# nebarnix/Project-Desert-Tortoise

Hardware: AMD Instinct MI355X
Metric: IQ Msamples/s end-to-end (WAV→minorframes), 1-GPU + %HBM roofline (higher is better)
Workload: dtype f32

## Files before the change

include/pdt_dev.h:

```cpp
#ifndef PDT_DEV_H
#define PDT_DEV_H
#include <stdint.h>
#ifdef __cplusplus
extern "C" {
#endif
int pdt_dev_set(const char *name, const char *value);
struct pdt_ctx;
unsigned long long pdt_dev_span_rows(const struct pdt_ctx *ctx, unsigned *n_exits_out, unsigned long long max);
unsigned long long pdt_dev_span_rekey(const struct pdt_ctx *ctx, unsigned *out, unsigned long long max);
unsigned pdt_dev_fir_form(const struct pdt_ctx *ctx, unsigned long long *fused_tiles_out);
int pdt_dev_ddc(int device, uint32_t in_rate, int decim, double offset_hz, int sample_format, const void *x_dev, long long lo, long long hi,
                uint64_t n_out, uint64_t g0, void *out_dev);
#ifdef __cplusplus
}
#endif
#endif
```

project-desert-tortoise_amd/__init__.py:

```python
from __future__ import annotations

import collections
import ctypes as C
import os
import struct

import numpy as np

_HERE = os.path.dirname(os.path.abspath(__file__))
LIBPDT_PATH = os.environ.get("PDT_LIBPDT_PATH") or os.path.join(_HERE, "csrc", "libpdt.so")
LIBSYNTH_PATH = os.path.join(_HERE, "synth", "libpdtsynth.so")

MODE_POES, MODE_ARGOS = 0, 1
SAMPLER_GARDNER, SAMPLER_MM = 0, 1
CHAIN_FILE, CHAIN_LIVE = 0, 1
ST_PLL, ST_LOCK, ST_FIR, ST_AGC, ST_SYM, ST_SYMIDX, ST_BITS, ST_BITSYM, ST_AGC_RAW, ST_ANALYTIC, ST_CHANNEL = range(11)
FMT_PCM16, FMT_F32, FMT_REAL_PCM16, FMT_REAL_F32 = range(4)


FMT_WB_PCM16, FMT_WB_F32, FMT_WB_CU8, FMT_WB_CS8 = range(16, 20)


class PdtError(RuntimeError):
    pass
# ... 503 lines not shown
    "pdt_demod_pcm16", "pdt_demod_device", "pdt_demod_f32", "pdt_demod_device_f32", "pdt_demod_batch_device", "pdt_num_frames", "pdt_frames", "pdt_get_stats",
    "pdt_format_frames", "pdt_read_stage", "pdt_stage_len", "pdt_kernel_times", "pdt_make_lpf",
    "pdt_wav_parse_header", "pdt_time_axis", "pdt_stage_bytesync", "pdt_tip_check", "pdt_tip_frames",
    "pdt_stream_begin", "pdt_stream_push_pcm16", "pdt_stream_push_f32", "pdt_stream_end", "pdt_stream_frames",
    "pdt_keep_quality", "pdt_chunk_reports", "pdt_stage_manchester", "pdt_stage_fir", "pdt_stage_agc", "pdt_stage_squelch", "pdt_stage_pll", "pdt_stage_gardner", "pdt_stage_static_gain", "pdt_stage_mm",
    "pdt_keep_presquelch", "pdt_keep_pll", "pdt_stage_bytesync_from", "pdt_demod_fd", "pdt_format_records", "pdt_stream_retained", "pdt_host_math", "pdt_get_device",
    "pdt_write_frames", "pdt_write_records", "pdt_demod_file", "pdt_set_loop_params", "pdt_set_progress",
    "pdt_set_real_input", "pdt_demod_real", "pdt_demod_device_real", "pdt_stream_push_real", "pdt_host_analytic",
    "pdt_set_channel", "pdt_demod_channel", "pdt_demod_device_channel", "pdt_demod_channels_device", "pdt_demod_channels", "pdt_stream_push_channel", "pdt_host_ddc",
    "pdt_survey", "pdt_survey_device", "pdt_survey_spectrum", "pdt_host_survey",
    "pdt_bursts", "pdt_bursts_device", "pdt_burst_carriers", "pdt_waterfall_rows", "pdt_bursts_shape", "pdt_burst_peaks", "pdt_host_bursts",
    "pdt_device_math", "pdt_device_math_layout",
    "pdt_burst_windows", "pdt_demod_windows_device", "pdt_demod_windows", "pdt_demod_windows_held",
    "pdt_tones", "pdt_tones_batch", "pdt_host_tones",
    "pdt_argos_messages", "pdt_argos_messages_batch", "pdt_stage_argos_messages", "pdt_host_argos_messages", "pdt_argos_msg_tile",
    "pdt_format_argos_messages", "pdt_write_argos_messages",
    "pdt_ff_bits", "pdt_ff_bits_batch", "pdt_ff_read", "pdt_ff_messages", "pdt_ff_messages_batch", "pdt_stage_ff_bits", "pdt_host_ff_bits",
    "pdt_host_ff_mix",
    "pdt_ffp_bits", "pdt_ffp_read", "pdt_ffp_blocks", "pdt_ffp_frames", "pdt_stage_ffp_bits", "pdt_stage_ffp_frames", "pdt_host_ffp_bits",
    "pdt_host_ffp_mix",
    "pdt_tip_sync", "pdt_tip_sync_batch", "pdt_stage_tip_sync", "pdt_host_tip_sync", "pdt_tip_sync_tile", "pdt_tip_check_records",
    "pdt_tip_repair", "pdt_stage_tip_repair", "pdt_host_tip_repair",
]
DEV_SYMBOLS = ["pdt_dev_set", "pdt_dev_span_rows", "pdt_dev_span_rekey", "pdt_dev_fir_form", "pdt_dev_ddc"]

_lib = None


def _share_torch_hip_runtime():
    import importlib.util
    import sys
    if "torch" in sys.modules:
        return
    try:
        spec = importlib.util.find_spec("torch")
    except (ImportError, ValueError):
        return
    if spec is None or not spec.submodule_search_locations:
        return
    path = os.path.join(list(spec.submodule_search_locations)[0], "lib", "libamdhip64.so")
    if os.path.exists(path):
        try:
            C.CDLL(path, mode=C.RTLD_GLOBAL)
        except OSError:
            pass


# ... 63 lines not shown
    L.pdt_stage_mm.argtypes = [C.c_void_p, C.c_void_p, C.c_uint64, C.c_void_p, C.c_void_p, C.c_void_p, C.c_void_p]
    L.pdt_stage_mm.restype = C.c_int
    L.pdt_stage_agc.argtypes = [C.c_void_p, C.c_void_p, C.c_uint64, C.c_double, C.c_double, C.c_double, C.c_void_p]
    L.pdt_stage_agc.restype = C.c_int
    L.pdt_stage_squelch.argtypes = [C.c_void_p, C.c_void_p, C.c_void_p, C.c_uint64, C.c_double]
    L.pdt_stage_squelch.restype = C.c_int
    L.pdt_stage_fir.argtypes = [C.c_void_p, C.c_void_p, C.c_uint64, C.c_void_p, C.c_void_p]
    L.pdt_stage_fir.restype = C.c_int
    L.pdt_keep_quality.argtypes = [C.c_void_p, C.c_int]
    L.pdt_keep_quality.restype = C.c_int
    L.pdt_keep_pll.argtypes = [C.c_void_p, C.c_int]
    L.pdt_keep_pll.restype = C.c_int
    L.pdt_chunk_reports.argtypes = [C.c_void_p, C.c_void_p, C.c_uint64]
    L.pdt_chunk_reports.restype = C.c_uint64
    L.pdt_set_progress.argtypes = [C.c_void_p, C.c_void_p, C.c_void_p]
    L.pdt_tip_check.argtypes = [C.c_void_p, C.POINTER(TipSummary)]
    L.pdt_tip_frames.argtypes = [C.c_void_p, C.c_void_p, C.c_uint64]
    L.pdt_tip_frames.restype = C.c_uint64
    L.pdt_write_frames.argtypes = [C.c_void_p, C.c_int, C.POINTER(C.c_uint64)]
    L.pdt_write_records.argtypes = [C.c_void_p, C.c_uint64, C.c_int, C.POINTER(C.c_uint64)]
    L.pdt_dev_set.argtypes = [C.c_char_p, C.c_char_p]
    L.pdt_dev_fir_form.argtypes = [C.c_void_p, C.POINTER(C.c_ulonglong)]
    L.pdt_dev_fir_form.restype = C.c_uint
    L.pdt_set_loop_params.argtypes = [C.c_void_p, C.POINTER(LoopParams)]
    L.pdt_demod_file.argtypes = [C.c_void_p, C.c_int, C.c_uint64, C.c_uint64, C.c_int, C.c_int, C.POINTER(C.c_uint64)]
    L.pdt_set_real_input.argtypes = [C.c_void_p, C.c_double]
    L.pdt_demod_real.argtypes = [C.c_void_p, C.c_void_p, C.c_uint64, C.c_int]
    L.pdt_demod_device_real.argtypes = [C.c_void_p, C.c_void_p, C.c_uint64, C.c_int]
    L.pdt_stream_push_real.argtypes = [C.c_void_p, C.c_void_p, C.c_uint64, C.c_int, C.POINTER(C.c_uint64)]
    L.pdt_host_analytic.argtypes = [C.c_uint32, C.c_double, C.c_void_p, C.c_uint64, C.c_int, C.c_void_p]
    L.pdt_set_channel.argtypes = [C.c_void_p, C.c_int, C.c_double]
    L.pdt_demod_channel.argtypes = [C.c_void_p, C.c_void_p, C.c_uint64, C.c_int]
    L.pdt_demod_device_channel.argtypes = [C.c_void_p, C.c_void_p, C.c_uint64, C.c_int]
    L.pdt_demod_channels_device.argtypes = [C.POINTER(C.c_void_p), C.c_int, C.c_void_p, C.c_uint64, C.c_int]
    L.pdt_demod_channels.argtypes = [C.POINTER(C.c_void_p), C.c_int, C.c_void_p, C.c_uint64, C.c_int]
    L.pdt_stream_push_channel.argtypes = [C.c_void_p, C.c_void_p, C.c_uint64, C.c_int, C.POINTER(C.c_uint64)]
    L.pdt_host_ddc.argtypes = [C.c_uint32, C.c_int, C.c_double, C.c_void_p, C.c_uint64, C.c_int, C.c_void_p]
    L.pdt_dev_ddc.argtypes = [C.c_int, C.c_uint32, C.c_int, C.c_double, C.c_int, C.c_void_p, C.c_longlong, C.c_longlong, C.c_uint64, C.c_uint64, C.c_void_p]
    L.pdt_survey.argtypes = [C.c_void_p, C.c_void_p, C.c_uint64, C.c_int, C.POINTER(SurveyCfg), C.POINTER(CarrierRec), C.c_int, C.POINTER(C.c_int)]
    L.pdt_survey_device.argtypes = L.pdt_survey.argtypes
    L.pdt_survey_spectrum.argtypes = [C.c_void_p, C.c_void_p, C.c_int]
    L.pdt_bursts.argtypes = [C.c_void_p, C.c_void_p, C.c_uint64, C.c_int, C.POINTER(BurstsCfg), C.POINTER(BurstRec), C.c_int, C.POINTER(C.c_int)]
    L.pdt_bursts_device.argtypes = L.pdt_bursts.argtypes
    L.pdt_burst_carriers.argtypes = [C.POINTER(BurstRec), C.c_int, C.c_double, C.POINTER(CarrierRec), C.c_int, C.POINTER(C.c_int)]
    L.pdt_waterfall_rows.argtypes = [C.c_void_p, C.c_uint64, C.c_uint64, C.c_void_p]
    L.pdt_bursts_shape.argtypes = [C.c_void_p, C.POINTER(C.c_int), C.POINTER(C.c_int), C.POINTER(C.c_uint64)]
# ... 523 lines not shown
        ns = C.c_uint64(0)
        _check(self._L.pdt_stage_mm(self._h, a.ctypes.data, a.size, C.addressof(state) if state is not None else None,
                                    sym.ctypes.data, pick.ctypes.data, C.addressof(ns)), "pdt_stage_mm")
        return sym[:ns.value], pick[:ns.value]

    def stage_agc(self, x: np.ndarray, initial: float, state: "AgcState | None" = None, attack: float = 0.0, decay: float = 0.0):
        a = np.array(x, dtype=self._dt(), copy=True)
        _check(self._L.pdt_stage_agc(self._h, a.ctypes.data, a.size, float(initial), float(attack), float(decay),
                                     C.addressof(state) if state is not None else None), "pdt_stage_agc")
        return a

    def stage_squelch(self, x: np.ndarray, lock: np.ndarray, threshold: float) -> np.ndarray:
        a = np.array(x, dtype=self._dt(), copy=True)
        l = np.ascontiguousarray(lock, dtype=self._dt())
        assert a.size == l.size
        _check(self._L.pdt_stage_squelch(self._h, a.ctypes.data, l.ctypes.data, a.size, float(threshold)), "pdt_stage_squelch")
        return a

    def fir_form(self) -> "tuple[int, int]":
        tiles = C.c_ulonglong(0)
        form = self._L.pdt_dev_fir_form(self._h, C.byref(tiles))
        return int(form), int(tiles.value)

    def stats_interp(self) -> int:
        taps, interp = make_lpf(self.mode, self.sample_rate)
        return int(interp)

    def frames(self) -> list[Frame]:
        n = self._L.pdt_num_frames(self._h)
        arr = (Frame * max(n, 1))()
        got = self._L.pdt_frames(self._h, arr, n)
        return [arr[i] for i in range(got)]

    def frames_array(self) -> np.ndarray:
        n = self._L.pdt_num_frames(self._h)
        buf = np.zeros(n, dtype=FRAME_DTYPE)
        if n:
            self._L.pdt_frames(self._h, C.cast(buf.ctypes.data, C.POINTER(Frame)), n)
        return buf

    def stats(self) -> Stats:
        s = Stats()
        _check(self._L.pdt_get_stats(self._h, C.byref(s)), "pdt_get_stats")
        return s

    def text(self) -> bytes:
# ... 265 lines not shown
```

project-desert-tortoise_amd/csrc/pdt_api.hip:

```cpp
#include "pdt_rt.h"
#include "pdt_analytic.h"
#include "pdt_ddc.h"
#include "pdt_survey.h"
#include "pdt_bursts.h"
#include "pdt_tone.h"
#include "pdt_argos_msg.h"
#include "pdt_tip_sync.h"
#include "pdt_ff.h"
#include "pdt_ffp.h"

#include <sys/stat.h>

namespace pdtrt {
PDT_CHAIN_INSTANCES(extern, float)
PDT_CHAIN_INSTANCES(extern, double)
std::atomic<long long> g_alloc_ns{0};
hipError_t analytic_launch(hipStream_t st, int fmt, const void *x, long long lo, long long hi, unsigned long long n_out, unsigned long long g0,
                           uint32_t step, const float *tab_dev, void *out);
size_t survey_part_floats(uint64_t nseg, int nfft);
hipError_t survey_launch(hipStream_t st, int fmt, const void *x, uint64_t nseg, int nfft, const float *win, const float *tw, float *part, float *out);
int survey_plan(const pdt_survey_cfg *cfg, double mode_range_hz, double channel_rate, uint64_t nframes, int cap, pdt::SurveyPlan *p);
int survey_carriers(const float *P, const pdt::SurveyPlan &p, double in_rate, pdt_carrier *found);
hipError_t waterfall_launch(hipStream_t st, int fmt, const void *x, uint64_t nrows, int rows_per, int nfft, const float *win, const float *tw, float *rows);
hipError_t row_peaks_launch(hipStream_t st, const float *rows, uint64_t nrows, int nfft, float level, int gb, void *peaks, int *counts);
// ... 21 lines not shown
               std::vector<uint32_t> &starts, pdt::FfpSync *head);
hipError_t tip_repair_launch(hipStream_t st, void *recs_dev, unsigned nrec, const float *soft_dev, const unsigned long long *nbits_dev, long long bit_cap,
                             void *info_dev, void *sum_dev);
long long ddc_windows_table(int decim, pdt::DdcWindow *win, int count, std::vector<unsigned char> &table);
hipError_t ddc_windows_launch(hipStream_t st, int fmt, int decim, const float *taps_dev, const float *tab_dev, const void *table_dev, int count,
                              long long tiles);
hipError_t ddc_launch(hipStream_t st, int fmt, int decim, const float *taps_dev, const float *tab_dev, pdt::DdcWindow w);
}

static std::mutex g_dev_mu;
static std::map<std::string, std::string> g_dev;
void Tuning::load()
{
    std::lock_guard<std::mutex> lock(g_dev_mu);
    if (g_dev.empty()) return;
    auto get = [&](const char *n) -> const char * { auto it = g_dev.find(n); return it == g_dev.end() ? nullptr : it->second.c_str(); };
    if (const char *e = get("PDT_PLL_WARM_SCALE")) pll_warm_scale = atof(e);
    if (const char *e = get("PDT_HEAD_TAUS")) head_taus = atof(e);
    if (const char *e = get("PDT_BAND_PAD")) band_pad = atof(e);
    if (const char *e = get("PDT_PLL_WARM_S")) pll_warm_s = atof(e);
    if (const char *e = get("PDT_AGC_WARM_S")) agc_warm_s = atof(e);
    if (const char *e = get("PDT_AGC_K")) agc_k = atof(e);
    if (const char *e = get("PDT_AGC_TPB")) agc_tpb = std::max(1, atoi(e));
    if (const char *e = get("PDT_PLL_BLOCK")) pll_block = atoi(e);
    if (const char *e = get("PDT_HBM_LIMIT_MB")) hbm_limit_mb = std::max(1ll, atoll(e));
    if (const char *e = get("PDT_BURST_SLAB_ROWS")) burst_slab_rows = std::max(1ll, atoll(e));
    if (const char *e = get("PDT_WINDOW_PIECE")) window_piece = std::max(1ll, atoll(e));
    if (const char *e = get("PDT_SCOUT_SYMS")) scout_syms = std::max(16, atoi(e));
    if (const char *e = get("PDT_FIR_WG_PER_CU")) fir_wg_per_cu = std::min(4096, std::max(1, atoi(e)));
    if (const char *e = get("PDT_INGEST_THREADS")) ingest_threads = std::min(128, std::max(1, atoi(e)));
    if (const char *e = get("PDT_INGEST_SPAN_MB")) ingest_span_mb = std::min(256, std::max(1, atoi(e)));
    if (const char *e = get("PDT_INGEST_STREAMS")) ingest_streams = std::min(4, std::max(1, atoi(e)));
    if (const char *e = get("PDT_INGEST_DIRECT")) ingest_direct = atoi(e) ? 1 : 0;
    if (const char *e = get("PDT_INGEST_NUMA")) ingest_numa = atoi(e) ? 1 : 0;
    if (const char *e = get("PDT_FIX_PASSES")) fix_passes = atoi(e);
    if (const char *e = get("PDT_GSEG")) gseg = std::min(64, std::max(2, atoi(e)));
    if (const char *e = get("PDT_GSPAN")) gspan = std::min(256, std::max(1, atoi(e)));
    if (const char *e = get("PDT_GSPAN_REKEY")) gspan_rekey = std::min(255, std::max(0, atoi(e)));
    if (const char *e = get("PDT_GSPAN_SUB")) gspan_sub = atoi(e);
    if (const char *e = get("PDT_GSPAN_WIN2")) gspan_win2 = atoi(e);
    if (const char *e = get("PDT_GSPAN_FIT")) gspan_fit = std::min(64, std::max(2, atoi(e)));
    if (const char *e = get("PDT_GSPAN_CAP")) gspan_cap = std::max(64, atoi(e));
    fir_generic = get("PDT_FIR_GENERIC") != nullptr;
    mix_unfused = get("PDT_MIX_UNFUSED") != nullptr;
    quality_inline = get("PDT_QUALITY_INLINE") != nullptr;
    gardner_nostride = get("PDT_GARDNER_NOSTRIDE") != nullptr;
// ... 228 lines not shown
    if (out && m) {
        const bool staged = ctx->gspan_rekey > 0 && ctx->gspan_info.p;
        std::vector<GardnerSpanRow> rows((size_t)m);
        std::vector<GardnerSpanRowInfo> info((size_t)m);
        if (hipSetDevice(ctx->cfg.device) != hipSuccess ||
            hipMemcpy(rows.data(), ctx->gspan_rows.p, (size_t)m * sizeof(GardnerSpanRow), hipMemcpyDeviceToHost) != hipSuccess ||
            (staged && hipMemcpy(info.data(), ctx->gspan_info.p, (size_t)m * sizeof(GardnerSpanRowInfo), hipMemcpyDeviceToHost) != hipSuccess)) {
            (void)hipGetLastError();
            return 0;
        }
        for (size_t k = 0; k < (size_t)m; k++) {
            out[3 * k] = rows[k].n;
            out[3 * k + 1] = staged ? info[k].states : 0u;
            out[3 * k + 2] = staged ? info[k].items : 0u;
        }
    }
    return n;
}

unsigned pdt_dev_fir_form(const pdt_ctx *ctx, unsigned long long *fused_tiles_out)
{
    if (fused_tiles_out) *fused_tiles_out = ctx ? (unsigned long long)ctx->fir_fused_tiles : 0ull;
    return ctx ? (unsigned)ctx->fir_form : 0u;
}

int pdt_dev_ddc(int device, uint32_t in_rate, int decim, double offset_hz, int sample_format, const void *x_dev, long long lo, long long hi,
                uint64_t n_out, uint64_t g0, void *out_dev)
{
    if (in_rate == 0 || decim < DDC_MIN_DECIM || decim > DDC_MAX_DECIM || !ddc_fmt(sample_format) || !x_dev || !out_dev) return PDT_ERR_ARG;
    if (!(std::isfinite(offset_hz) && std::fabs(offset_hz) < 0.5 * (double)in_rate)) return PDT_ERR_ARG;
    HIP_TRY(hipSetDevice(device));
    const std::vector<float> taps = ddc_taps(decim);
    std::vector<float> tab(2 * AN_TAB);
    analytic_table(tab.data());
    DevBuf dtaps, dtab;
    auto run = [&]() -> int {
        int rc;
        if ((rc = dtaps.ensure(taps.size() * sizeof(float) + 16)) || (rc = dtab.ensure(tab.size() * sizeof(float) + 16))) return rc;
        HIP_TRY(hipMemcpy(dtaps.p, taps.data(), taps.size() * sizeof(float), hipMemcpyHostToDevice));
        HIP_TRY(hipMemcpy(dtab.p, tab.data(), tab.size() * sizeof(float), hipMemcpyHostToDevice));
        const DdcWindow r = { x_dev, out_dev, lo, hi, (long long)n_out, ddc_step((double)in_rate, offset_hz), (uint32_t)g0, 0 };
        HIP_TRY(ddc_launch(nullptr, sample_format, decim, (const float *)dtaps.p, (const float *)dtab.p, r));
        HIP_TRY(hipStreamSynchronize(nullptr));
        return PDT_OK;
    };
    const int rc = run();
// ... 2676 lines not shown
```

project-desert-tortoise_amd/csrc/pdt_chain.inc:

```
#include "pdt_rt.h"

namespace pdtrt {
PDT_WIDE_INSTANCES(extern, float)
PDT_WIDE_INSTANCES(extern, double)

template <typename T> int finish_capture(pdt_ctx *ctx, uint64_t n, const FinishArgs &FA)
{
    const bool argos = FA.argos, need_lock = FA.need_lock, fuse_mix = FA.fuse_mix;
    const long long N = FA.N, n_out = FA.n_out, chunk = FA.chunk, chunk_out = FA.chunk_out, first = FA.first, first_out = FA.first_out,
                    sym_cap = FA.sym_cap;
    const int interp = FA.interp, ntaps = FA.ntaps;
    const uint32_t hit_cap = FA.hit_cap, frame_cap = FA.frame_cap;
    const SyncParams &SP = FA.SP;
    const T Fs = (T)ctx->cfg.sample_rate;
    StreamCarry *seg = ctx->sc.active ? &ctx->sc : nullptr;
    FrameRec *d_frames = (FrameRec *)ctx->frames.p;
    (void)first_out;
    if (!ctx->pending || ctx->pend_n != n) return PDT_ERR_STATE;
    ctx->pending = false;
    pdt_ctx *lead = ctx->leader ? ctx->leader : ctx;
    if (seg && seg->in_place && !ctx->tune.sync_block) {
        for (;;) {
            const hipError_t e = hipEventQuery(lead->ev1);
            if (e == hipSuccess) break;
// ... 243 lines not shown

    collect_timers();
    if (ctx->progress_fn && !ctx->chunk_host.empty()) {
        try {
            std::vector<pdt_chunk_report> rep(ctx->chunk_host.size());
            chunk_reports_range(ctx, 0, rep.size(), ctx->report_samples, rep.data(), nullptr);
            ctx->progress_fn(ctx->progress_user, 0, rep.data(), rep.size(), &ctx->stats);
        } catch (const std::bad_alloc &) {
            return PDT_ERR_NOMEM;
        }
    }
    return PDT_OK;
}


inline void agc_block_warm(const pdt_ctx *ctx, long long *Ba, long long *Wa)
{
    const bool argos = ctx->cfg.mode == PDT_MODE_ARGOS;
    const double fs_d = (double)ctx->cfg.sample_rate;
    const int interp = (int)ctx->interp;
    auto round4 = [](long long v) { return (v + 3) / 4 * 4; };
    *Ba = std::max<long long>(64, round4(ctx->cfg.agc_block ? ctx->cfg.agc_block : (long long)((argos ? 0.125 : 0.0625) * fs_d * interp)));
    *Wa = round4(ctx->cfg.agc_warm ? ctx->cfg.agc_warm : (long long)((argos ? 2.0 : 8.0) * fs_d * interp));
}

template <typename T> void rec_static_gain(Plan &PL, hipStream_t st, IqSrc src, long long n, T *mag, T level, double norm_override, T *d_norm)
{
    PDT_LAUNCH(256, k_static_gain<T>, dim3(1), dim3(256), 0, st, src, n, mag, level, norm_override, d_norm);
}

template <typename T> void rec_squelch(Plan &PL, hipStream_t st, T *data, const T *lock, long long n, T thr)
{
    PDT_LAUNCH(256, k_squelch<T>, dim3((unsigned)((n + 1023) / 1024)), dim3(256), 0, st, data, lock, n, thr);
}

template <typename T> bool rec_fir_unfused(pdt_ctx *ctx, Plan &PL, hipStream_t st, const T *d_in, long long N, T *d_out, AgcMap *tile_maps, T agc_decay)
{
    const bool argos = ctx->cfg.mode == PDT_MODE_ARGOS;
    const int interp = (int)ctx->interp, ntaps = (int)ctx->ntaps;
    const T *d_taps = (const T *)ctx->taps.p;
    const int opt = 8;
    const long long tile = (long long)PDT_FIR_THREADS * opt;
    const long long grid = (N * interp + tile - 1) / tile;
    if (argos) {
        const size_t sh = (size_t)(ntaps + tile + ntaps + 8) * sizeof(T);
        PDT_LAUNCH(PDT_FIR_THREADS, k_fir_plain<T>, dim3((unsigned)grid), dim3(PDT_FIR_THREADS), sh, st, d_in, N, ntaps, d_taps, d_out, opt);
// ... 265 lines not shown
        Wacq = (long long)(0.02 * fs_d);
        agc_block_warm(ctx, &Ba, &Wa);
        if (argos && !ctx->cfg.agc_block && ctx->batch_hint >= 8) Ba = (long long)(1.0 * fs_d * interp);
        if (!ctx->cfg.pll_block) {
            const long long groups_max = ctx->batch_hint > 1 ? 240 : 150;
            const long long share = std::max<long long>(1, groups_max / std::max(1, ctx->batch_hint));
            const long long b_min = (N + share * 256 - 1) / (share * 256);
            Bp = std::max(Bp, b_min);
        }
        Bp = std::min<long long>(Bp, std::max<long long>(N, 1));
        Bp = std::max<long long>(64, (Bp + 63) / 64 * 64);
        seg_fast = seg && first_out % PDT_MF_RUN == 0 && first_out % 32 == 0 && !ctx->tune.seg_plain;
        fuse_mix = false;
        if constexpr (std::is_same<T, float>::value) {
            fuse_mix = !argos && !live && !inject && (!seg || seg_fast) && interp == 1 && ntaps == 26 && ctx->taps_rot.p && !ctx->tune.fir_generic &&
                       !ctx->tune.mix_unfused && N >= 832;
            if (fuse_mix && !ctx->cfg.pll_block) Bp = (Bp + 831) / 832 * 832;
            if (fuse_mix && Bp % 832 != 0) fuse_mix = false;
        }
        Ba = std::max<long long>(64, round4(Ba));
        agc_tiles_per_block = 0;
        fused_tiles = 0;
        agc_maps_per_block = 0;
        if (!argos && !ctx->cfg.agc_block && ntaps == 26 * interp && ctx->taps_rot.p && !ctx->tune.fir_generic &&
            !ctx->tune.agc_unfused && (!seg || (seg_fast && first_out % (64ll * 26 * interp) == 0) || (seg_fast && fuse_mix))) {
            const long long tile_out = 64ll * 26 * interp;
            agc_tiles_per_block = std::max<long long>(1, (Ba + tile_out / 2) / tile_out);
            {
                const long long tiles = (n_out - first_out + tile_out - 1) / tile_out;
                const long long one_round = (tiles + 500ll * 64 - 1) / (500ll * 64);
                if (ctx->batch_hint <= 1 && tiles / agc_tiles_per_block > 512ll * 64 && one_round <= 4 * agc_tiles_per_block)
                    agc_tiles_per_block = one_round;
            }
            if (ctx->tune.agc_tpb) agc_tiles_per_block = ctx->tune.agc_tpb;
            Ba = agc_tiles_per_block * tile_out;
        }
        Wp = round4(Wp);
        Wa = round4(Wa);
        Wacq = round4(Wacq);
        sym_rate = (double)baud;
        f_lim = (double)PP.max_freq * fs_d / (2.0 * M_PI);
        lag = (int)ceil(fs_d / sym_rate);
        lag = std::max(1, std::min(lag, (int)(fs_d / (2.2 * f_lim))));
        lag = std::min(lag, 64);
        nb_pll = N / Bp + 2;
        nb_agc = (n_out - first_out + Ba - 1) / Ba + 1;

        return PDT_OK;
    }

    int allocate()
    {
        int rc = PDT_OK;
        (void)rc;
        min_step = (double)GP.step - 0.25;
        if (ctx->cfg.sampler == PDT_SAMPLER_MM) {
            if ((rc = make_mm_params<T>(ctx, n_out, chunk_out, nullptr))) return rc;
// ... 385 lines not shown
                    else PDT_LAUNCH(512, (k_mix_fir<26, 1, 8, true>), dim3(mf_grid), dim3(512), 0, st, PDT_MF_ARGS, d_tap, mf_pll_from);
                } else {
                    if (d_pcm.fmt == 0) PDT_LAUNCH(512, (k_mix_fir<26, 0, 8>), dim3(mf_grid), dim3(512), 0, st, PDT_MF_ARGS, (float *)nullptr, mf_pll_from);
                    else PDT_LAUNCH(512, (k_mix_fir<26, 1, 8>), dim3(mf_grid), dim3(512), 0, st, PDT_MF_ARGS, (float *)nullptr, mf_pll_from);
                }
#undef PDT_MF_ARGS
                done = true;
            }
            if (!done) done = rec_fir_unfused<T>(ctx, PL, st, (const T *)d_pll, N, d_fir, fir_tile_maps, AP.decay);
            if (!done) fused_tiles = 0;
            ctx->fir_form = fuse_mix ? 2 : done ? 3 : argos ? 1 : 4;
            L.end();
        }
        ctx->fir_fused_tiles = fused_tiles;

        return PDT_OK;
    }

    int rec_agc()
    {
        int rc = PDT_OK;
        (void)rc;
        agc_last_block = -1;
        if (n_out - first_out > 0) {
            const long long na = n_out - first_out;
            const T *a_in = d_fir + first_out;
            T *a_out = d_agc + first_out;
            const T *a_lock = d_lock ? d_lock + first_out : nullptr;
            AgcParams<T> APs = AP;
            if (APs.raw_out) APs.raw_out += first_out;
            const long long nb = (na + Ba - 1) / Ba;
            agc_last_block = nb - 1;
            const bool fused = fused_tiles > 0;
            if (!fused && (rc = ctx->agc_maps.ensure((size_t)(nb + 1) * (sizeof(AgcMap) + sizeof(double))))) return rc;
            AgcMap *d_maps = (AgcMap *)ctx->agc_maps.p;
            double *d_guess = (double *)(d_maps + (fused ? fused_tiles : nb) + 1);
            const long long map_len_fused = fuse_mix ? (long long)PDT_MF_RUN : 64ll * 26 * interp;
            const long long map_first = fused ? first_out / map_len_fused : 0;
            const AgcMap *d_maps_in = d_maps + map_first;
            const long long n_maps_in = fused ? fused_tiles - map_first : nb;
            if (quality_side && !quality_term_fused) PL.simple(OP_JOIN_WAIT);
            L.begin("agc_block");
            if (agc_maps_per_block == 0) agc_maps_per_block = agc_tiles_per_block;
            if (fused && agc_maps_per_block > 1) {
                AgcMap *d_bmaps = (AgcMap *)(d_guess + nb + 1);
                PDT_LAUNCH(256, k_agc_blockmaps, dim3((unsigned)((nb + 255) / 256)), dim3(256), 0, st, d_maps_in, nb,
                                   (int)agc_maps_per_block, n_maps_in, d_bmaps);
                PDT_LAUNCH(1024, k_agc_guess<T>, dim3(1), dim3(1024), 0, st, (const AgcMap *)d_bmaps, nb, (const T *)d_norm, d_guess, 1, nb);
            } else if (fused)
                PDT_LAUNCH(1024, k_agc_guess<T>, dim3(1), dim3(1024), 0, st, d_maps_in, nb, (const T *)d_norm, d_guess, (int)agc_maps_per_block, n_maps_in);
            bool agc_tr = false;
            float *agc_ckpt = nullptr;
            if constexpr (std::is_same<T, float>::value) {
                agc_tr = fused && !ctx->tune.agc_lanes && !APs.squelch && !APs.raw_out && first_out % 32 == 0 && Ba % 32 == 0 &&
                         agc_maps_per_block > 0 && Ba % agc_maps_per_block == 0;
                if (agc_tr) {
                    const long long tile_len = 64ll * 26 * interp;
                    const long long map_len = Ba / agc_maps_per_block;
                    agc_tr = tile_len % 32 == 0 && tile_len % map_len == 0 && Ba % tile_len == 0;
                    if (agc_tr) {
                        const double agc_K = ctx->tune.agc_k > 0 ? ctx->tune.agc_k : 12.0;
                        const size_t ck_bytes = (size_t)(nb + 64) * (size_t)(Ba / PDT_AGC_CKPT + 1) * sizeof(float);
                        if ((rc = ctx->agc_ckpt.ensure(ck_bytes))) return rc;
                        agc_ckpt = (float *)ctx->agc_ckpt.p;
                        PDT_LAUNCH(64, (k_agc_block_tr<PDT_AGC_TR_R>), dim3((unsigned)((nb + 63) / 64)), dim3(64), 0, st, (const float *)a_in, na, APs,
                                   (const float *)d_norm, Ba, Wa, (const double *)d_guess, d_maps_in, (int)agc_maps_per_block,
                                   (int)(tile_len / map_len), n_maps_in, tile_len, (float *)a_out, (AgcSeam<float> *)ctx->seams_agc.p, agc_K, agc_ckpt);
                    }
                }
            }
            T *agc_ckpt_any = (T *)agc_ckpt;
            if (!agc_tr && (rc = rec_agc_lanes<T>(ctx, PL, st, a_in, na, APs, d_norm, Ba, Wa, !fused, d_maps, d_guess, a_lock, a_out, &agc_ckpt_any))) return rc;
            L.end();
            L.begin("agc_fix");
            rec_agc_fix<T>(ctx, PL, st, a_in, na, APs, Ba, a_lock, a_out, d_sc, agc_ckpt_any);
            L.end();
        }

        return PDT_OK;
    }

    int sampler_domain()
    {
        int rc = PDT_OK;
        (void)rc;
        use_mm = ctx->cfg.sampler == PDT_SAMPLER_MM;
        use_table = false;
        GD.q_min = 0; GD.u = 0; GD.n_q = 0; GD.n_cand = 0; GD.pad_q = 0; GD.idx_bits = 20; GD.span = 1;
        span_rekey = 0;
        if constexpr (std::is_same<T, float>::value) {
// ... 775 lines not shown
```

project-desert-tortoise_amd/csrc/pdt_kernels_front.h:

```cpp
#pragma once
#include <type_traits>
#include <utility>
#include "pdt_device_math.h"

namespace pdt {

template <typename T> struct PllParams {
    T Fs;
    T lock_thr;
    T lock_alpha;
    T alpha_acq, beta_acq, alpha_trk, beta_trk;
    T alpha_wide, beta_wide;
    T max_freq, min_freq;
    T sweep0, avg0, phase0;
    T freq0, locksig0;
    long long i0;
    T cond_lo, cond_hi;
    int want_lock;
};

template <typename T> struct PllState {
    T phase, freq, avg_phase, locksig, sweep;
};

// ... 2376 lines not shown
            __syncthreads();
            if ((int)threadIdx.x >= d) {
                Bc = A * Bp + Bc;
                A = A * Ap;
                sA[threadIdx.x] = A;
                sB[threadIdx.x] = Bc;
            }
            __syncthreads();
        }
        if (threadIdx.x == 0) {
            const double tA = sA[255], tB = sB[255];
            runB = tA * runB + tB;
            runA = tA * runA;
        }
    }
    if (threadIdx.x == 0) {
        AgcMap m;
        m.A = runA;
        m.B = runB;
        maps[j] = m;
    }
}

__device__ __forceinline__ void k_agc_blockmaps(const AgcMap *__restrict__ maps, long long nb, int maps_per_block, long long n_maps,
                                                AgcMap *__restrict__ bmaps)
{
    const long long j = (long long)blockIdx.x * blockDim.x + threadIdx.x;
    if (j >= nb) return;
    AgcMap bm;
    bm.A = 1.0; bm.B = 0.0;
    for (int q = 0; q < maps_per_block; q++) {
        const long long t = j * maps_per_block + q;
        if (t < n_maps) {
            const AgcMap m = maps[t];
            bm.B = m.A * bm.B + m.B;
            bm.A = m.A * bm.A;
        }
    }
    bmaps[j] = bm;
}

template <typename T>
__device__ __forceinline__ void k_agc_guess(const AgcMap *__restrict__ maps, long long nb, const T *__restrict__ norm,
                                                     double *__restrict__ guesses, int maps_per_block, long long n_maps)
{
    __shared__ double sA[1024], sB[1024];
    const long long per = (nb + 1023) / 1024;
    long long j0 = (long long)threadIdx.x * per, j1 = j0 + per;
    if (j0 > nb) j0 = nb;
    if (j1 > nb) j1 = nb;
    auto block_map = [&](long long j) {
        AgcMap bm;
        bm.A = 1.0; bm.B = 0.0;
        for (int q = 0; q < maps_per_block; q++) {
            const long long t = j * maps_per_block + q;
            if (t < n_maps) {
                const AgcMap m = maps[t];
                bm.B = m.A * bm.B + m.B;
                bm.A = m.A * bm.A;
            }
        }
        return bm;
    };
    double A = 1.0, Bc = 0.0;
    for (long long j = j0; j < j1; j++) {
        const AgcMap m = block_map(j);
        Bc = m.A * Bc + m.B;
        A = m.A * A;
    }
    sA[threadIdx.x] = A;
    sB[threadIdx.x] = Bc;
    __syncthreads();
    for (int d = 1; d < 1024; d <<= 1) {
        double Ap = 1.0, Bp = 0.0;
        if ((int)threadIdx.x >= d) { Ap = sA[threadIdx.x - d]; Bp = sB[threadIdx.x - d]; }
        __syncthreads();
        if ((int)threadIdx.x >= d) {
            Bc = A * Bp + Bc;
            A = A * Ap;
            sA[threadIdx.x] = A;
            sB[threadIdx.x] = Bc;
        }
        __syncthreads();
    }
    double Ae = 1.0, Be = 0.0;
    if (threadIdx.x > 0) { Ae = sA[threadIdx.x - 1]; Be = sB[threadIdx.x - 1]; }
    double g = Ae * (double)*norm + Be;
    for (long long j = j0; j < j1; j++) {
        double gg = g;
        if (!(gg > 1e-4)) gg = 1e-4;
        if (gg > 5000.0) gg = 5000.0;
        guesses[j] = gg;
        const AgcMap m = block_map(j);
        g = m.A * g + m.B;
    }
}

#define PDT_AGC_CKPT 1024
template <typename T>
__device__ __forceinline__ void k_agc_block(const T *__restrict__ in, long long n, AgcParams<T> P,
                                                   const T *__restrict__ norm, long long B, long long W,
                                                   const double *__restrict__ guesses, const T *__restrict__ lock,
                                                   T *__restrict__ out, AgcSeam<T> *__restrict__ seams, double K,
                                                   T *__restrict__ ckpt )
{
    __shared__ __attribute__((aligned(16))) unsigned char ring[PDT_AGC_PF * PDT_RING_SLOT];
    const long long j = (long long)blockIdx.x * blockDim.x + threadIdx.x;
    const long long start = j * B;
    if (start >= n) return;
    const long long end = (start + B < n) ? start + B : n;
    long long ws = 0;
    T gain = *norm;
    if (j >= 1) {
        const double g_here = guesses[j];
        double need = K * g_here / (double)P.decay;
        if (need < 4096.0) need = 4096.0;
        if (need > (double)W) need = (double)W;
        long long m = (long long)((need + (double)B - 1.0) / (double)B);
// ... 4 lines not shown
            gain = (T)g0;
        }
    }
    agc_range<T, false>(in, lock, out, ws, start, gain, P, ring);
    AgcSeam<T> sm;
    sm.g0 = gain;
    if (ckpt) {
        const long long ncp = B / PDT_AGC_CKPT;
        long long at = start;
        for (long long c = 0; c < ncp && at + PDT_AGC_CKPT <= end; c++, at += PDT_AGC_CKPT) {
            agc_range<T, true>(in, lock, out, at, at + PDT_AGC_CKPT, gain, P, ring);
            ckpt[j * ncp + c] = gain;
        }
        agc_range<T, true>(in, lock, out, at, end, gain, P, ring);
    } else
        agc_range<T, true>(in, lock, out, start, end, gain, P, ring);
    sm.g1 = gain;
    seams[j] = sm;
}

#define PDT_TR_SLOT 1040
#define PDT_TR_SB (8 * PDT_TR_SLOT)
#ifndef PDT_AGC_TR_R
#define PDT_AGC_TR_R 4
#endif
typedef float pdt_f4 __attribute__((ext_vector_type(4)));

template <bool STORE, bool PARTIAL, bool CLAMP, int R>
__device__ __forceinline__ void agc_range_tr(const float *__restrict__ in, float *__restrict__ out, long long e0, int rel0, long long nsb,
                                             float &gain, int from, const AgcParams<float> &P, unsigned char *ring,
                                             const unsigned (&voff)[8], long long n, long long B, long long jb0,
                                             float *__restrict__ ckpt = nullptr)
{
    const int t = threadIdx.x & 63;
    const unsigned ring0 = (unsigned)(size_t)ring;
    const unsigned char *mine = ring + (t & 7) * PDT_TR_SLOT + (t >> 3) * 128;
    unsigned char *stage_mine = ring + R * PDT_TR_SB + (t & 7) * PDT_TR_SLOT + (t >> 3) * 128;
    const unsigned char *stage_row = ring + R * PDT_TR_SB + t * 16;
    const char *gin = (const char *)(in + e0);
    char *gout = (char *)(out + e0);
    auto issue = [&](long long sb, int slot) {
        const char *b = gin + sb * 128;
#pragma unroll
        for (int s = 0; s < 8; s++) {
            unsigned vo = voff[s];
            if (CLAMP) {
                const long long e = e0 + sb * 32;
// ... 87 lines not shown
    const long long j = jb0 + t;
    const long long start = j * B;
    const bool valid = start < n;
    unsigned voff[8];
#pragma unroll
    for (int s = 0; s < 8; s++) {
        long long b = 8 * (t >> 3) + s;
        if ((jb0 + b) * B >= n) b = 0;
        voff[s] = (unsigned)((b * B + 4 * (t & 7)) * 4);
    }
    long long ws = 0;
    float gain = *norm;
    if (valid && j >= 1) {
        const double g_here = guesses[j];
        double need = K * g_here / (double)P.decay;
        if (need < 4096.0) need = 4096.0;
        if (need > (double)W) need = (double)W;
        const long long m = (long long)((need + (double)tile_len - 1.0) / (double)tile_len);
        const long long q = (start - m * tile_len) / tile_len;
        if (start - m * tile_len > 0 && q >= 1) {
            ws = q * tile_len;
            const long long jb = ws / B;
            double g = guesses[jb];
            for (long long u = jb * maps_per_block; u < q * maps_per_tile; u++)
                if (u < n_maps) {
                    const AgcMap mp = tmaps[u];
                    g = mp.A * g + mp.B;
                }
            if (!(g > 1e-4)) g = 1e-4;
            if (g > 5000.0) g = 5000.0;
            gain = (float)g;
        }
    }
    const bool partial = (jb0 + 64) * B > n;
    int back = valid ? (int)(start - ws) : 0;
#pragma unroll
    for (int d = 32; d >= 1; d >>= 1) {
        const int o = __shfl_xor(back, d);
        back = back > o ? back : o;
    }
    back = __builtin_amdgcn_readfirstlane(back);
    const int from = valid ? -(int)(start - ws) : 0x7fffffff;
    if (back > 0) {
        if (jb0 * B >= back) agc_range_tr<false, false, false, R>(in, out, jb0 * B - back, -back, back / 32, gain, from, P, ring, voff, n, B, jb0);
        else agc_range_tr<false, false, true, R>(in, out, jb0 * B - back, -back, back / 32, gain, from, P, ring, voff, n, B, jb0);
    }
    AgcSeam<float> sm;
    sm.g0 = gain;
    float *my_ckpt = (ckpt && valid) ? ckpt + j * (B / PDT_AGC_CKPT) : nullptr;
    if (!partial) agc_range_tr<true, false, false, R>(in, out, jb0 * B, 0, B / 32, gain, 0, P, ring, voff, n, B, jb0, my_ckpt);
    else agc_range_tr<true, true, false, R>(in, out, jb0 * B, 0, B / 32, gain, 0, P, ring, voff, n, B, jb0, my_ckpt);
// ... 73 lines not shown
```

project-desert-tortoise_amd/csrc/pdt_rt.h:

```cpp
#ifndef PDT_RT_H
#define PDT_RT_H
#include <hip/hip_runtime.h>
#include <math.h>
#include <stdio.h>
#include <stdlib.h>
#include <string.h>

#include <errno.h>
#include <fcntl.h>
#include <unistd.h>

#include <algorithm>
#include <functional>
#include <map>
#include <mutex>
#include <atomic>
#include <chrono>
#include <memory>
#include <new>
#include <string>
#include <thread>
#include <type_traits>
#include <vector>

#include "../../include/pdt.h"
#include "../../include/pdt_dev.h"
#include "pdt_kernels_back.h"
#include "pdt_kernels_front.h"
#include "pdt_timeaxis.h"
#include "pdt_ingest.h"
#include "pdt_work_layout.h"

using namespace pdt;

#define HIP_TRY(expr)                                                                                  \
    do {                                                                                               \
        hipError_t e_ = (expr);                                                                        \
        if (e_ != hipSuccess) {                                                                        \
            fprintf(stderr, "libpdt: %s failed: %s (%s:%d)\n", #expr, hipGetErrorString(e_), __FILE__, \
                    __LINE__);                                                                         \
            return PDT_ERR_NOGPU;                                                                      \
        }                                                                                              \
    } while (0)

namespace pdtrt {

extern std::atomic<long long> g_alloc_ns;
struct AllocTimer {
    std::chrono::steady_clock::time_point t0 = std::chrono::steady_clock::now();
    ~AllocTimer() { g_alloc_ns += std::chrono::duration_cast<std::chrono::nanoseconds>(std::chrono::steady_clock::now() - t0).count(); }
};
inline hipError_t timed_host_malloc(void **p, size_t bytes)
{
    AllocTimer t;
// ... 175 lines not shown
    bool same_shape(const Plan &o) const
    {
        if (ops.size() != o.ops.size() || packs.size() != o.packs.size()) return false;
        for (size_t i = 0; i < ops.size(); i++) {
            const PlanOp &a = ops[i], &b = o.ops[i];
            if (a.op != b.op || a.side != b.side || a.go != b.go || a.block.x != b.block.x || a.block.y != b.block.y ||
                a.shmem != b.shmem || a.pack_off != b.pack_off || a.pack_size != b.pack_size)
                return false;
        }
        return true;
    }
};
#define PDT_LAUNCH(TB, KERNEL, grid, block, shmem, stream, ...) \
    PL.launch<&KERNEL, TB>(#KERNEL, grid, block, shmem, PL.side_of(stream), __VA_ARGS__)

}
using namespace pdtrt;

struct Tuning {
    double band_pad = 0.0, pll_warm_scale = 1.0, head_taus = 0.0, agc_k = 0.0, pll_warm_s = 0.0, agc_warm_s = 0.0;
    double overlap_split[8] = { 0, 0, 0, 0, 0, 0, 0, 0 };
    long long hbm_limit_mb = 0, window_piece = 0, burst_slab_rows = 0;
    int ingest_direct = -1, ingest_numa = -1;
    int scout_syms = 0, gspan = 0, gspan_cap = 0, gspan_rekey = -1 , gspan_sub = 0, gspan_win2 = 0, gspan_fit = 0, ingest_threads = 0, ingest_span_mb = 0, ingest_streams = 0, overlap_segments = 0, overlap_min_mb = 0, fir_wg_per_cu = 0, agc_tpb = 0, gseg = 0, pll_block = 0, fix_passes = 2;
    bool fir_generic = false, mix_unfused = false, quality_inline = false, gemit_groups = false, agc_unfused = false, no_excl = false, gardner_onebuf = false, gardner_noring = false, gardner_sequential = false, seg_sequential = false, agc_lanes = false, overlap = true, debug_overlap = false, chain_one_range = false, ema_noguess = false, debug_sync = false, pll_noshort = false, pll_nockpt = false, pll_noconsensus = false, pll_notail = false, seg_plain = false, sync_block = false, gardner_nostride = false, manch_3pass = false, sync_serial = false;
    void load();
};

struct StreamCarry {
    bool active = false;
    bool final_seg = false;
    bool in_place = false;
    uint64_t place_align = 0;
    bool quality = false;
    long long first = 0;
    uint64_t origin = 0;
    bool have_norm = false;
    double norm_factor = 0, gain = 0;
    bool locked = false;
    double phase = 0, freq = 0, avg = 0, locksig = 0, sweep = 0;
    int64_t lock_sample = -1;
    double lock_freq_hz = 0, avg_at_lock = 0;
    bool have_sampler = false;
    double sa = 0, sb = 0, sc = 0;
    double sym_m2 = 0, sym_m1 = 0;
    unsigned clockmod = 0;
    uint64_t nsym_total = 0;
// ... 64 lines not shown
    bool keep_agc_raw = false;
    bool keep_quality = false;
    bool keep_pll_asked = false;
    bool keep_pll = true;
    DevBuf avgph, term_ap, seams_q, chunkinfo;
    struct PllInject {
        bool active = false, started = false, locked = false;
        double phase = 0, freq = 0, avg = 0, locksig = 0, sweep = 0;
    } inj;
    long long last_pll_block = 0;
    void *qual_pin = nullptr;
    size_t qual_pin_cap = 0;
    uint64_t pend_chunks = 0;
    std::vector<pdt::ChunkInfo> chunk_host;
    uint64_t report_samples = 0;
    pdt_progress_fn progress_fn = nullptr;
    void *progress_user = nullptr;
    long long gcand_key = -1;
    int gardner_mode = 0;
    long long gspan_nrows = 0;
    int gspan_rekey = 0;
    int fir_form = 0;
    long long fir_fused_tiles = 0;
    const void *pcm_dev = nullptr;
    int pcm_fmt = 0;

    std::vector<unsigned char> taps_host;
    uint64_t n_samples = 0, n_out = 0;
    std::vector<pdt_frame> frames_host;
    std::vector<pdt_tip_frame> tip_host;
    uint32_t frames_on_device = 0;
    bool have_frames = false;
    Plan plan;
    DevBuf packs_dev;
    void *packs_pin = nullptr;
    size_t packs_pin_cap = 0;
    pdt_ctx *leader = nullptr;
    int batch_hint = 1;
    IngestRes ingest;
    double stream_gpu_ms = 0;
    double ingest_ms = 0;
    DevBuf stream_in, seg_dev, lt_theta, lt_phi;
    uint64_t stream_have = 0, stream_done = 0;
    uint64_t stream_total = 0;
    int stream_fmt = -1;
    bool stream_open = false;
    std::vector<pdt_frame> stream_new;
    uint32_t real_step = 1u << 30;
    double real_center = 0;
    DevBuf an_tab, analytic;
    int an_tab_ready = 0;
    uint64_t analytic_len = 0;
    int ch_decim = 0;
    double ch_offset = 0;
    uint32_t ch_step = 0;
    DevBuf ddc_taps, channel;
    int ddc_taps_decim = 0;
    uint64_t channel_len = 0;
    HaloCarry halo;
    DevBuf survey_win, survey_tw, survey_part, survey_out;
    int survey_tab_nfft = 0;
// ... 388 lines not shown
```

Measured before the change: 55270.

## Size AGC tiles-per-block from device LDS occupancy and shrink transpose ring depth

Sets the AGC tiles-per-block split from queried CU count and LDS capacity, taking walkers per round from the kernel's static LDS size. It replaces the hard-coded 500/512×64 lane heuristic. The default transpose ring depth drops from 4 to 3, adding a runtime switch that instantiates depths 3–5. Map-composition loops are batched eight loads at a time. The aim is a better-balanced single-round AGC sweep with more resident workgroups, at the cost of less prefetch depth per walker.

Result: no change. 55350, median of 4 (+0.2%).

```diff
diff --git a/include/pdt_dev.h b/include/pdt_dev.h
--- a/include/pdt_dev.h
+++ b/include/pdt_dev.h
@@ -9,6 +9,7 @@
 unsigned long long pdt_dev_span_rows(const struct pdt_ctx *ctx, unsigned *n_exits_out, unsigned long long max);
 unsigned long long pdt_dev_span_rekey(const struct pdt_ctx *ctx, unsigned *out, unsigned long long max);
 unsigned pdt_dev_fir_form(const struct pdt_ctx *ctx, unsigned long long *fused_tiles_out);
+unsigned pdt_dev_agc_form(const struct pdt_ctx *ctx, unsigned long long *tiles_per_block_out, unsigned long long *walkers_out);
 int pdt_dev_ddc(int device, uint32_t in_rate, int decim, double offset_hz, int sample_format, const void *x_dev, long long lo, long long hi,
                 uint64_t n_out, uint64_t g0, void *out_dev);
 #ifdef __cplusplus
diff --git a/project-desert-tortoise_amd/__init__.py b/project-desert-tortoise_amd/__init__.py
--- a/project-desert-tortoise_amd/__init__.py
+++ b/project-desert-tortoise_amd/__init__.py
@@ -549,7 +549,7 @@
     "pdt_tip_sync", "pdt_tip_sync_batch", "pdt_stage_tip_sync", "pdt_host_tip_sync", "pdt_tip_sync_tile", "pdt_tip_check_records",
     "pdt_tip_repair", "pdt_stage_tip_repair", "pdt_host_tip_repair",
 ]
-DEV_SYMBOLS = ["pdt_dev_set", "pdt_dev_span_rows", "pdt_dev_span_rekey", "pdt_dev_fir_form", "pdt_dev_ddc"]
+DEV_SYMBOLS = ["pdt_dev_set", "pdt_dev_span_rows", "pdt_dev_span_rekey", "pdt_dev_fir_form", "pdt_dev_agc_form", "pdt_dev_ddc"]
 
 _lib = None
 
@@ -659,6 +659,8 @@
     L.pdt_dev_set.argtypes = [C.c_char_p, C.c_char_p]
     L.pdt_dev_fir_form.argtypes = [C.c_void_p, C.POINTER(C.c_ulonglong)]
     L.pdt_dev_fir_form.restype = C.c_uint
+    L.pdt_dev_agc_form.argtypes = [C.c_void_p, C.POINTER(C.c_ulonglong), C.POINTER(C.c_ulonglong)]
+    L.pdt_dev_agc_form.restype = C.c_uint
     L.pdt_set_loop_params.argtypes = [C.c_void_p, C.POINTER(LoopParams)]
     L.pdt_demod_file.argtypes = [C.c_void_p, C.c_int, C.c_uint64, C.c_uint64, C.c_int, C.c_int, C.POINTER(C.c_uint64)]
     L.pdt_set_real_input.argtypes = [C.c_void_p, C.c_double]
@@ -1228,6 +1230,11 @@
         form = self._L.pdt_dev_fir_form(self._h, C.byref(tiles))
         return int(form), int(tiles.value)
 
+    def agc_form(self) -> "tuple[int, int, int]":
+        tpb, walkers = C.c_ulonglong(0), C.c_ulonglong(0)
+        ring = self._L.pdt_dev_agc_form(self._h, C.byref(tpb), C.byref(walkers))
+        return int(ring), int(tpb.value), int(walkers.value)
+
     def stats_interp(self) -> int:
         taps, interp = make_lpf(self.mode, self.sample_rate)
         return int(interp)
diff --git a/project-desert-tortoise_amd/csrc/pdt_agc_geometry.h b/project-desert-tortoise_amd/csrc/pdt_agc_geometry.h
--- /dev/null
+++ b/project-desert-tortoise_amd/csrc/pdt_agc_geometry.h
@@ -0,0 +1,36 @@
+#ifndef PDT_AGC_GEOMETRY_H
+#define PDT_AGC_GEOMETRY_H
+
+namespace pdtrt {
+
+enum { AGC_SIMDS_PER_CU = 4, AGC_LANES = 64 };
+
+inline long long agc_walkers_per_cu(long long lds_per_cu, long long lds_per_wg)
+{
+    if (lds_per_wg <= 0) return AGC_SIMDS_PER_CU;
+    const long long fit = lds_per_cu / lds_per_wg;
+    return fit < 0 ? 0 : fit > AGC_SIMDS_PER_CU ? AGC_SIMDS_PER_CU : fit;
+}
+
+enum { AGC_WALKERS_PER_CU_PACED = 2 };
+
+inline long long agc_walkers_per_round(long long cus, long long lds_per_cu, long long lds_per_wg)
+{
+    const long long fit = agc_walkers_per_cu(lds_per_cu, lds_per_wg);
+    return cus <= 0 ? 0 : cus * (fit > AGC_WALKERS_PER_CU_PACED ? AGC_WALKERS_PER_CU_PACED : fit);
+}
+
+inline long long agc_tiles_per_block(long long walkers, long long tiles, long long tpb_default, long long forced)
+{
+    if (forced > 0) return forced;
+    if (tpb_default < 1) tpb_default = 1;
+    if (walkers <= 0 || tiles <= 0) return tpb_default;
+    const long long lanes_full = walkers * AGC_LANES;
+    const long long lanes = walkers * 125 / 128 * AGC_LANES > 0 ? walkers * 125 / 128 * AGC_LANES : lanes_full;
+    const long long one_round = (tiles + lanes - 1) / lanes;
+    if (tiles / tpb_default > lanes_full && one_round <= 4 * tpb_default) return one_round;
+    return tpb_default;
+}
+
+}
+#endif
diff --git a/project-desert-tortoise_amd/csrc/pdt_api.hip b/project-desert-tortoise_amd/csrc/pdt_api.hip
--- a/project-desert-tortoise_amd/csrc/pdt_api.hip
+++ b/project-desert-tortoise_amd/csrc/pdt_api.hip
@@ -67,6 +67,7 @@
     if (const char *e = get("PDT_AGC_WARM_S")) agc_warm_s = atof(e);
     if (const char *e = get("PDT_AGC_K")) agc_k = atof(e);
     if (const char *e = get("PDT_AGC_TPB")) agc_tpb = std::max(1, atoi(e));
+    if (const char *e = get("PDT_AGC_RING")) agc_ring = std::min(5, std::max(3, atoi(e)));
     if (const char *e = get("PDT_PLL_BLOCK")) pll_block = atoi(e);
     if (const char *e = get("PDT_HBM_LIMIT_MB")) hbm_limit_mb = std::max(1ll, atoll(e));
     if (const char *e = get("PDT_BURST_SLAB_ROWS")) burst_slab_rows = std::max(1ll, atoll(e));
@@ -341,6 +342,13 @@
 {
     if (fused_tiles_out) *fused_tiles_out = ctx ? (unsigned long long)ctx->fir_fused_tiles : 0ull;
     return ctx ? (unsigned)ctx->fir_form : 0u;
+}
+
+unsigned pdt_dev_agc_form(const pdt_ctx *ctx, unsigned long long *tiles_per_block_out, unsigned long long *walkers_out)
+{
+    if (tiles_per_block_out) *tiles_per_block_out = ctx ? (unsigned long long)ctx->agc_form_tpb : 0ull;
+    if (walkers_out) *walkers_out = ctx ? (unsigned long long)ctx->agc_form_walkers : 0ull;
+    return ctx ? (unsigned)ctx->agc_form_ring : 0u;
 }
 
 int pdt_dev_ddc(int device, uint32_t in_rate, int decim, double offset_hz, int sample_format, const void *x_dev, long long lo, long long hi,
diff --git a/project-desert-tortoise_amd/csrc/pdt_chain.inc b/project-desert-tortoise_amd/csrc/pdt_chain.inc
--- a/project-desert-tortoise_amd/csrc/pdt_chain.inc
+++ b/project-desert-tortoise_amd/csrc/pdt_chain.inc
@@ -289,6 +289,34 @@
     auto round4 = [](long long v) { return (v + 3) / 4 * 4; };
     *Ba = std::max<long long>(64, round4(ctx->cfg.agc_block ? ctx->cfg.agc_block : (long long)((argos ? 0.125 : 0.0625) * fs_d * interp)));
     *Wa = round4(ctx->cfg.agc_warm ? ctx->cfg.agc_warm : (long long)((argos ? 2.0 : 8.0) * fs_d * interp));
+}
+
+static_assert(PDT_AGC_TR_R >= 3 && PDT_AGC_TR_R <= 5, "k_agc_block_tr is instantiated for ring depths 3, 4 and 5");
+inline int agc_ring_depth(const pdt_ctx *ctx) { return ctx->tune.agc_ring ? ctx->tune.agc_ring : PDT_AGC_TR_R; }
+
+template <int R> long long agc_tr_static_lds()
+{
+    hipFuncAttributes fa;
+    if (hipFuncGetAttributes(&fa, reinterpret_cast<const void *>(&k_run<&k_agc_block_tr<R>, 64>)) != hipSuccess) {
+        (void)hipGetLastError();
+        return (long long)(R + 1) * PDT_TR_SB;
+    }
+    return (long long)fa.sharedSizeBytes;
+}
+template <typename T> long long agc_round_walkers(pdt_ctx *ctx, int R)
+{
+    if (!std::is_same<T, float>::value) R = 0;
+    long long &have = ctx->agc_round_walkers[R ? R - 2 : 0];
+    if (have > 0) return have;
+    int cus = 0, lds_cu = 0, lds_wg = 0;
+    if (hipDeviceGetAttribute(&cus, hipDeviceAttributeMultiprocessorCount, ctx->cfg.device) != hipSuccess) { (void)hipGetLastError(); cus = 0; }
+    if (hipDeviceGetAttribute(&lds_cu, hipDeviceAttributeMaxSharedMemoryPerMultiprocessor, ctx->cfg.device) != hipSuccess) { (void)hipGetLastError(); lds_cu = 0; }
+    if (hipDeviceGetAttribute(&lds_wg, hipDeviceAttributeMaxSharedMemoryPerBlock, ctx->cfg.device) != hipSuccess) { (void)hipGetLastError(); lds_wg = 0; }
+    long long lds = (long long)PDT_AGC_PF * PDT_RING_SLOT;
+    if constexpr (std::is_same<T, float>::value)
+        lds = R == 3 ? agc_tr_static_lds<3>() : R == 4 ? agc_tr_static_lds<4>() : R == 5 ? agc_tr_static_lds<5>() : lds;
+    have = agc_walkers_per_round(cus, std::max(lds_cu, lds_wg), lds);
+    return have;
 }
 
 template <typename T> void rec_static_gain(Plan &PL, hipStream_t st, IqSrc src, long long n, T *mag, T level, double norm_override, T *d_norm)
@@ -600,17 +628,19 @@
         agc_tiles_per_block = 0;
         fused_tiles = 0;
         agc_maps_per_block = 0;
+        ctx->agc_form_walkers = 0;
         if (!argos && !ctx->cfg.agc_block && ntaps == 26 * interp && ctx->taps_rot.p && !ctx->tune.fir_generic &&
             !ctx->tune.agc_unfused && (!seg || (seg_fast && first_out % (64ll * 26 * interp) == 0) || (seg_fast && fuse_mix))) {
             const long long tile_out = 64ll * 26 * interp;
             agc_tiles_per_block = std::max<long long>(1, (Ba + tile_out / 2) / tile_out);
             {
                 const long long tiles = (n_out - first_out + tile_out - 1) / tile_out;
-                const long long one_round = (tiles + 500ll * 64 - 1) / (500ll * 64);
-                if (ctx->batch_hint <= 1 && tiles / agc_tiles_per_block > 512ll * 64 && one_round <= 4 * agc_tiles_per_block)
-                    agc_tiles_per_block = one_round;
-            }
-            if (ctx->tune.agc_tpb) agc_tiles_per_block = ctx->tune.agc_tpb;
+                bool lines = false;
+                if constexpr (std::is_same<T, float>::value) lines = !seg && !ctx->tune.agc_lanes && !ctx->keep_agc_raw;
+                const long long walkers = ctx->batch_hint <= 1 ? agc_round_walkers<T>(ctx, lines ? agc_ring_depth(ctx) : 0) : 0;
+                agc_tiles_per_block = pdtrt::agc_tiles_per_block(walkers, tiles, agc_tiles_per_block, ctx->tune.agc_tpb);
+                ctx->agc_form_walkers = walkers;
+            }
             Ba = agc_tiles_per_block * tile_out;
         }
         Wp = round4(Wp);
@@ -1042,6 +1072,8 @@
         int rc = PDT_OK;
         (void)rc;
         agc_last_block = -1;
+        ctx->agc_form_ring = 0;
+        ctx->agc_form_tpb = agc_tiles_per_block;
         if (n_out - first_out > 0) {
             const long long na = n_out - first_out;
             const T *a_in = d_fir + first_out;
@@ -1083,9 +1115,17 @@
                         const size_t ck_bytes = (size_t)(nb + 64) * (size_t)(Ba / PDT_AGC_CKPT + 1) * sizeof(float);
                         if ((rc = ctx->agc_ckpt.ensure(ck_bytes))) return rc;
                         agc_ckpt = (float *)ctx->agc_ckpt.p;
-                        PDT_LAUNCH(64, (k_agc_block_tr<PDT_AGC_TR_R>), dim3((unsigned)((nb + 63) / 64)), dim3(64), 0, st, (const float *)a_in, na, APs,
-                                   (const float *)d_norm, Ba, Wa, (const double *)d_guess, d_maps_in, (int)agc_maps_per_block,
-                                   (int)(tile_len / map_len), n_maps_in, tile_len, (float *)a_out, (AgcSeam<float> *)ctx->seams_agc.p, agc_K, agc_ckpt);
+#define PDT_AGC_TR_LAUNCH(R)                                                                                                                        \
+    PDT_LAUNCH(64, (k_agc_block_tr<R>), dim3((unsigned)((nb + 63) / 64)), dim3(64), 0, st, (const float *)a_in, na, APs, (const float *)d_norm, Ba, \
+               Wa, (const double *)d_guess, d_maps_in, (int)agc_maps_per_block, (int)(tile_len / map_len), n_maps_in, tile_len, (float *)a_out,     \
+               (AgcSeam<float> *)ctx->seams_agc.p, agc_K, agc_ckpt)
+                        ctx->agc_form_ring = agc_ring_depth(ctx);
+                        switch (ctx->agc_form_ring) {
+                        case 3: PDT_AGC_TR_LAUNCH(3); break;
+                        case 5: PDT_AGC_TR_LAUNCH(5); break;
+                        default: PDT_AGC_TR_LAUNCH(4); break;
+                        }
+#undef PDT_AGC_TR_LAUNCH
                     }
                 }
             }
diff --git a/project-desert-tortoise_amd/csrc/pdt_kernels_front.h b/project-desert-tortoise_amd/csrc/pdt_kernels_front.h
--- a/project-desert-tortoise_amd/csrc/pdt_kernels_front.h
+++ b/project-desert-tortoise_amd/csrc/pdt_kernels_front.h
@@ -2422,6 +2422,21 @@
     }
 }
 
+template <typename F>
+__device__ __forceinline__ void agc_maps_each(const AgcMap *__restrict__ maps, long long u0, long long u1, long long n_maps, F &&apply)
+{
+    if (u1 > n_maps) u1 = n_maps;
+    long long u = u0;
+    for (; u + 8 <= u1; u += 8) {
+        AgcMap m[8];
+#pragma unroll
+        for (int k = 0; k < 8; k++) m[k] = maps[u + k];
+#pragma unroll
+        for (int k = 0; k < 8; k++) apply(m[k]);
+    }
+    for (; u < u1; u++) apply(maps[u]);
+}
+
 __device__ __forceinline__ void k_agc_blockmaps(const AgcMap *__restrict__ maps, long long nb, int maps_per_block, long long n_maps,
                                                 AgcMap *__restrict__ bmaps)
 {
@@ -2429,14 +2444,10 @@
     if (j >= nb) return;
     AgcMap bm;
     bm.A = 1.0; bm.B = 0.0;
-    for (int q = 0; q < maps_per_block; q++) {
-        const long long t = j * maps_per_block + q;
-        if (t < n_maps) {
-            const AgcMap m = maps[t];
-            bm.B = m.A * bm.B + m.B;
-            bm.A = m.A * bm.A;
-        }
-    }
+    agc_maps_each(maps, j * maps_per_block, (j + 1) * maps_per_block, n_maps, [&](const AgcMap &m) {
+        bm.B = m.A * bm.B + m.B;
+        bm.A = m.A * bm.A;
+    });
     bmaps[j] = bm;
 }
 
@@ -2462,12 +2473,15 @@
         }
         return bm;
     };
+    const bool plain = maps_per_block == 1;
     double A = 1.0, Bc = 0.0;
-    for (long long j = j0; j < j1; j++) {
-        const AgcMap m = block_map(j);
+    auto compose = [&](const AgcMap &m) {
         Bc = m.A * Bc + m.B;
         A = m.A * A;
-    }
+    };
+    if (plain) agc_maps_each(maps, j0, j1, n_maps, compose);
+    else
+        for (long long j = j0; j < j1; j++) compose(block_map(j));
     sA[threadIdx.x] = A;
     sB[threadIdx.x] = Bc;
     __syncthreads();
@@ -2486,14 +2500,21 @@
     double Ae = 1.0, Be = 0.0;
     if (threadIdx.x > 0) { Ae = sA[threadIdx.x - 1]; Be = sB[threadIdx.x - 1]; }
     double g = Ae * (double)*norm + Be;
-    for (long long j = j0; j < j1; j++) {
+    long long j = j0;
+    auto put = [&](const AgcMap &m) {
         double gg = g;
         if (!(gg > 1e-4)) gg = 1e-4;
         if (gg > 5000.0) gg = 5000.0;
-        guesses[j] = gg;
-        const AgcMap m = block_map(j);
+        guesses[j++] = gg;
         g = m.A * g + m.B;
-    }
+    };
+    if (plain) {
+        agc_maps_each(maps, j0, j1, n_maps, put);
+        AgcMap id;
+        id.A = 1.0; id.B = 0.0;
+        while (j < j1) put(id);
+    } else
+        while (j < j1) put(block_map(j));
 }
 
 #define PDT_AGC_CKPT 1024
@@ -2544,7 +2565,7 @@
 #define PDT_TR_SLOT 1040
 #define PDT_TR_SB (8 * PDT_TR_SLOT)
 #ifndef PDT_AGC_TR_R
-#define PDT_AGC_TR_R 4
+#define PDT_AGC_TR_R 3
 #endif
 typedef float pdt_f4 __attribute__((ext_vector_type(4)));
 
@@ -2678,11 +2699,7 @@
             ws = q * tile_len;
             const long long jb = ws / B;
             double g = guesses[jb];
-            for (long long u = jb * maps_per_block; u < q * maps_per_tile; u++)
-                if (u < n_maps) {
-                    const AgcMap mp = tmaps[u];
-                    g = mp.A * g + mp.B;
-                }
+            agc_maps_each(tmaps, jb * maps_per_block, q * maps_per_tile, n_maps, [&](const AgcMap &mp) { g = mp.A * g + mp.B; });
             if (!(g > 1e-4)) g = 1e-4;
             if (g > 5000.0) g = 5000.0;
             gain = (float)g;
diff --git a/project-desert-tortoise_amd/csrc/pdt_rt.h b/project-desert-tortoise_amd/csrc/pdt_rt.h
--- a/project-desert-tortoise_amd/csrc/pdt_rt.h
+++ b/project-desert-tortoise_amd/csrc/pdt_rt.h
@@ -30,6 +30,7 @@
 #include "pdt_timeaxis.h"
 #include "pdt_ingest.h"
 #include "pdt_work_layout.h"
+#include "pdt_agc_geometry.h"
 
 using namespace pdt;
 
@@ -251,7 +252,7 @@
     double overlap_split[8] = { 0, 0, 0, 0, 0, 0, 0, 0 };
     long long hbm_limit_mb = 0, window_piece = 0, burst_slab_rows = 0;
     int ingest_direct = -1, ingest_numa = -1;
-    int scout_syms = 0, gspan = 0, gspan_cap = 0, gspan_rekey = -1 , gspan_sub = 0, gspan_win2 = 0, gspan_fit = 0, ingest_threads = 0, ingest_span_mb = 0, ingest_streams = 0, overlap_segments = 0, overlap_min_mb = 0, fir_wg_per_cu = 0, agc_tpb = 0, gseg = 0, pll_block = 0, fix_passes = 2;
+    int scout_syms = 0, gspan = 0, gspan_cap = 0, gspan_rekey = -1 , gspan_sub = 0, gspan_win2 = 0, gspan_fit = 0, ingest_threads = 0, ingest_span_mb = 0, ingest_streams = 0, overlap_segments = 0, overlap_min_mb = 0, fir_wg_per_cu = 0, agc_tpb = 0, agc_ring = 0 , gseg = 0, pll_block = 0, fix_passes = 2;
     bool fir_generic = false, mix_unfused = false, quality_inline = false, gemit_groups = false, agc_unfused = false, no_excl = false, gardner_onebuf = false, gardner_noring = false, gardner_sequential = false, seg_sequential = false, agc_lanes = false, overlap = true, debug_overlap = false, chain_one_range = false, ema_noguess = false, debug_sync = false, pll_noshort = false, pll_nockpt = false, pll_noconsensus = false, pll_notail = false, seg_plain = false, sync_block = false, gardner_nostride = false, manch_3pass = false, sync_serial = false;
     void load();
 };
@@ -362,6 +363,8 @@
     int gspan_rekey = 0;
     int fir_form = 0;
     long long fir_fused_tiles = 0;
+    int agc_form_ring = 0;
+    long long agc_form_tpb = 0, agc_form_walkers = 0;
     const void *pcm_dev = nullptr;
     int pcm_fmt = 0;
 
@@ -377,6 +380,7 @@
     size_t packs_pin_cap = 0;
     pdt_ctx *leader = nullptr;
     int batch_hint = 1;
+    long long agc_round_walkers[4] = { 0, 0, 0, 0 };
     IngestRes ingest;
     double stream_gpu_ms = 0;
     double ingest_ms = 0;
```
